# crismolav/ggnn

Measured on AMD Instinct MI355X. Metric: instances/sec (graphs/s) GGNN fwd+bwd, hidden=256 v=128 e=4 T=5, higher is better.
Workload: dtype fp32; 1 GPU; configs[2]: b=256 graphs/GPU, v=128, hidden=256, e=4 (C=8), T=5, fwd+bwd; global_batch=256, parallelism=dp1

## Files before the change

ggnn_amd/csrc/ggnn_api.hip:

```cpp
#include <hip/hip_runtime.h>
#include <stdint.h>
#include <string.h>

#include <algorithm>
#include <cmath>
#include <string>
#include <vector>

#include "../../include/ggnn.h"
#include "ggnn_common.h"
#include "k_gru.h"
#include "k_gru2.h"
#include "k_fused.h"
#include "k_prep.h"
#include "k_prop.h"
#include "k_optim.h"
#include "k_wgrad.h"
#include "k_head.h"
#include "k_decode.h"
#include "k_tree.h"
#include "k_proj.h"
#include "k_marg.h"
#include "k_lapl.h"
#include "k_tree_loss.h"
// ... 450 lines not shown
  Prof p(K_GRU_BWD, s);
  *nwg = (int)(c.N / (32 * RT));
  hipLaunchKernelGGL((k_gru_bwd<H, RT, PREC>), dim3(c.N / (32 * RT)), dim3(2 * H), 0, s, delta, hf, r, u, cc,
                     P<u16>(pk, PL.WcT), P<u16>(pk, PL.WgT), PL.loWc, PL.loWg, (ActT<PREC>*)dXT, dh_out,
                     (u16*)dzcT, (u16*)dzgT, dbc, dbg, c.N, gmax, bpart,
                     (H == 256 && c.V == 128) ? sbits : (const uint2*)nullptr, c.sdrop.scale);
}
long gru_bias_rows(const Cfg& c) { return (long)c.T * std::max<long>(c.N / 32, 1); }

#define DISPATCH_V(c, FN, H, PREC, ...)                 \
  do {                                                  \
    if ((c).V == 32) FN<32, H, PREC>(__VA_ARGS__);      \
    else if ((c).V == 64) FN<64, H, PREC>(__VA_ARGS__); \
    else FN<128, H, PREC>(__VA_ARGS__);                 \
  } while (0)
#define DISPATCH_VH(c, FN, PREC, ...)                                  \
  do {                                                                 \
    if ((c).H == 64) DISPATCH_V(c, FN, 64, PREC, __VA_ARGS__);         \
    else if ((c).H == 128) DISPATCH_V(c, FN, 128, PREC, __VA_ARGS__);  \
    else DISPATCH_V(c, FN, 256, PREC, __VA_ARGS__);                    \
  } while (0)
#define DISPATCH_RT(c, FN, H, PREC, ...)                                             \
  do {                                                                               \
    constexpr bool sp_ = Prec<PREC>::split;                                          \
    constexpr int mx_ = sp_ ? kSplitRT<FN##_tag>::value : kMaxRT<FN##_tag, H>::value; \
    const int rt_ = gru_rt(c, mx_);                                                  \
    if (mx_ >= 4 && rt_ == 4) FN<H, mx_ >= 4 ? 4 : 2, PREC>(__VA_ARGS__);            \
    else if (rt_ == 2) FN<H, 2, PREC>(__VA_ARGS__);                                  \
    else FN<H, 1, PREC>(__VA_ARGS__);                                                \
  } while (0)
#define DISPATCH_HRT(c, FN, PREC, ...)                                 \
  do {                                                                 \
    if ((c).H == 64) DISPATCH_RT(c, FN, 64, PREC, __VA_ARGS__);        \
    else if ((c).H == 128) DISPATCH_RT(c, FN, 128, PREC, __VA_ARGS__); \
    else DISPATCH_RT(c, FN, 256, PREC, __VA_ARGS__);                   \
  } while (0)

struct launch_gru_fwd_tag {};
struct launch_gru_bwd_tag {};
template <typename TAG, int H> struct kMaxRT { static constexpr int value = 4; };
template <typename TAG> struct kSplitRT { static constexpr int value = 2; };
template <> struct kMaxRT<launch_gru_bwd_tag, 256> { static constexpr int value = 2; };

void launch_pack(bool f16, const float* S, int ldS, long sS, int K, int N, int trans, u16* out, long sO, long lo,
                 int batch, hipStream_t s, Drop dr = Drop{0, 0, 0, 1.0f}, int t = 0) {
  const int total = (N / 32) * (K / 16) * 64;
  Prof p(K_PACK, s);
  if (f16)
    hipLaunchKernelGGL(k_pack_B<true>, dim3((total + 255) / 256, batch), dim3(256), 0, s, S, ldS, sS, K, N, trans, out,
                       sO, lo, dr, t);
  else
    hipLaunchKernelGGL(k_pack_B<false>, dim3((total + 255) / 256, batch), dim3(256), 0, s, S, ldS, sS, K, N, trans, out,
                       sO, lo, dr, t);
}
const Drop kNoDrop = {0, 0, 0, 1.0f};

template <int PREC>
int forward_impl(const Cfg& c, const void* pack, const void* adj, void* ws, bool tr, const float* h0, float* hT,
                 hipStream_t s) {
  typedef ActT<PREC> Act;
  constexpr bool SPLIT = Prec<PREC>::split;
  const WsL L = ws_layout(c, tr);
  const PackL PL = pack_layout(c);
  const AdjL AL = adj_layout(c);
  const long N = c.N, H = c.H;
  const bool dense = c.vin == c.V;
  const bool fused = fused_fwd(c);
  float* hf0 = tr ? P<float>(ws, L.hfT) : P<float>(ws, L.hf[0]);
  if (tr) {
    Prof p(K_IO, s);
    hipLaunchKernelGGL((k_stage_h0<Prec<PREC>::f16>), dim3((N + 63) / 64, H / 64), dim3(256), 0, s, h0, c.vin, c.V,
                       hf0, SPLIT ? (u16*)nullptr : P<u16>(ws, L.hb[0]), P<u16>(ws, L.hT), N, c.H);
  } else if (!dense || (!SPLIT && !fused)) {
    Prof p(K_IO, s);
    hipLaunchKernelGGL(k_pad_state, dim3(grid1d(N / 4 * H)), dim3(256), 0, s, h0, c.vin, c.V, c.H,
                       dense ? (float*)nullptr : hf0, SPLIT ? (u16*)nullptr : P<u16>(ws, L.hb[0]), N,
                       (int)Prec<PREC>::f16, kNoDrop, 0, (const uint32_t*)nullptr);
  }
  if (fused) {
    FusedFwdArgs fa;
    memset(&fa, 0, sizeof(fa));
    fa.Ab = P<u16>(adj, AL.Ab);
    const ChanL cl = chan_lists(c, adj, AL);
    fa.chl = cl.p;
    fa.chs = cl.stride;
    fa.Wp = P<u16>(pack, PL.wf(0));
    fa.wlo = PL.loW;
    fa.wstep = c.ed ? (long)(PL.szW / 2) : 0;
    fa.beta = P<float>(pack, PL.beta);
    fa.Wgp = P<u16>(pack, PL.Wg);
    fa.bg = P<float>(pack, PL.bg);
    fa.Wcp = P<u16>(pack, PL.Wc);
    fa.bc = P<float>(pack, PL.bc);
    fa.wlo_g = PL.loWg;
    fa.wlo_c = PL.loWc;
    fa.Xs = P<float>(ws, L.Xa);
    for (int t = 0; t <= c.T; ++t) {
      const float* hin = tr ? P<float>(ws, L.hfT + L.nh4 * t) : (t == 0 && dense) ? h0 : P<float>(ws, L.hf[t & 1]);
      fa.hf[t] = (t == c.T && dense) ? hT : (float*)hin;
    }
    if (tr) {
      fa.XT = P<u16>(ws, L.XT);
      fa.hT = P<u16>(ws, L.hT);
      fa.rhT = P<u16>(ws, L.rhT);
      fa.r = P<float>(ws, L.r);
      fa.u = P<float>(ws, L.u);
      fa.c = P<float>(ws, L.c);
      fa.sw = (long)(L.nhw / 2);
      fa.s4 = (long)(L.nh4 / 4);
    }
    fa.C = c.C;
    fa.T = c.T;
    fa.vsh = c.vsh;
    fa.sd = c.sdrop;
    fa.sbits = (tr && state_bits(c)) ? P<uint2>(ws, L.sbits) : nullptr;
    {
      Prof p(K_FWD_FUSED, s);
      hipLaunchKernelGGL(k_fwd_fused<PREC>, dim3(c.b), dim3(512), 0, s, fa);
    }
  } else
  for (int t = 0; t < c.T; ++t) {
    const float* hf_in = tr ? P<float>(ws, L.hfT + L.nh4 * t)
                            : (t == 0 && dense) ? h0 : P<float>(ws, L.hf[t & 1]);
    float* hf_out = (t + 1 == c.T && dense) ? hT
                    : tr                   ? P<float>(ws, L.hfT + L.nh4 * (t + 1))
                                           : P<float>(ws, L.hf[(t + 1) & 1]);
    const u16* hb_in = SPLIT ? nullptr : P<u16>(ws, L.hb[t & 1]);
    u16* hb_out = SPLIT ? nullptr : P<u16>(ws, L.hb[(t + 1) & 1]);
    const void* hs = SPLIT ? (const void*)hf_in : (const void*)hb_in;
    void* XT = tr ? P<void>(ws, L.XT + L.nhw * t) : nullptr;
    DISPATCH_VH(c, launch_prop_fwd, PREC, c, t, hs, P<u16>(adj, AL.Ab), chan_lists(c, adj, AL), PL, pack,
                P<void>(ws, L.Xa), XT, s);
    void* hTo = (tr && t + 1 < c.T) ? P<void>(ws, L.hT + L.nhw * (t + 1)) : nullptr;
    float* ro = tr ? P<float>(ws, L.r + L.nh4 * t) : nullptr;
    float* uo = tr ? P<float>(ws, L.u + L.nh4 * t) : nullptr;
    float* co = tr ? P<float>(ws, L.c + L.nh4 * t) : nullptr;
    void* rhT = tr ? P<void>(ws, L.rhT + L.nhw * t) : nullptr;
    DISPATCH_HRT(c, launch_gru_fwd, PREC, c, t, P<void>(ws, L.Xa), hb_in, hf_in, PL, pack, hf_out, hb_out, hTo, ro, uo,
                 co, rhT, s);
  }
  const float* hfin = tr ? P<float>(ws, L.hfT + L.nh4 * c.T) : P<float>(ws, L.hf[c.T & 1]);
  if (!dense) {
    Prof p(K_IO, s);
    hipLaunchKernelGGL(k_unpad_state, dim3(grid1d((long)c.b * c.vin * H)), dim3(256), 0, s, hfin, c.vin, c.V, c.H, hT,
                       (long)c.b, (const uint32_t*)nullptr);
  }
  LAUNCHCHK();
  return GGNN_OK;
}

template <int PREC>
int wgrad_impl(const Cfg& c, void* ws, int t0, int nt, float* dW, float* dWg, float* dWc, hipStream_t s);

struct Zeroer {
  hipStream_t s;
  ZeroJobs j;
  int n = 0;
  explicit Zeroer(hipStream_t st) : s(st) {}
  void add(float* p, long cnt) {
    if (cnt <= 0) return;
    j.p[n] = p, j.n[n] = cnt;
    if (++n == ZERO_MAXJ) flush();
  }
  void flush() {
    if (n) hipLaunchKernelGGL(k_zero_multi, dim3(256, n), dim3(256), 0, s, j);
    n = 0;
  }
  ~Zeroer() { flush(); }
};

template <int PREC>
int backward_impl(const Cfg& c, const void* pack, const void* adj, void* ws, const float* dhT, float* dh0, float* dW,
                  float* dbeta, float* dWg, float* dbg, float* dWc, float* dbc, hipStream_t s) {
  const WsL L = ws_layout(c, true);
  const PackL PL = pack_layout(c);
  const AdjL AL = adj_layout(c);
  const long N = c.N, H = c.H;
  const bool use_bias = (c.flags & GGNN_USE_EDGE_BIAS) != 0;
  if (H < 128) return fail(GGNN_EUNSUP, "weight gradients need hidden >= 128");

  const uint32_t* gmax = P<const uint32_t>(ws, L.gmax);
  {
    Prof p(K_IO, s);
    absmax(dhT, (long)c.b * c.vin * H, P<uint32_t>(ws, L.gmax), s);
  }
  float* dA = P<float>(ws, L.dA);
  float* dB = P<float>(ws, L.dB);
  const bool dense = c.vin == c.V;
  const uint2* sb = state_bits(c) ? P<const uint2>(ws, L.sbits) : nullptr;
  const bool in_place = dense && (!c.sd || sb);
  if (!in_place) {
    Prof p(K_IO, s);
    hipLaunchKernelGGL(k_pad_state, dim3(grid1d(N / 4 * H)), dim3(256), 0, s, dhT, c.vin, c.V, c.H, dA, (u16*)nullptr, N, 0,
                       c.sdrop, c.T - 1, gmax);
  }
  const long gb_stride = std::max<long>(N / 32, 1);
  int gb_nwg = 0;
  for (int t = c.T - 1; t >= 0; --t) {
    const bool first = t == c.T - 1 && in_place, last = t == 0 && dense;
    const float* delta = first ? dhT : dA;
    float* dh_out = last ? dh0 : dA;
// ... 99 lines not shown
  if (N % KC) return fail(GGNN_EUNSUP, "rows not divisible into weight-gradient chunks");
  a.KC = KC;
  a.nchunks = (int)(N / KC);
  {
    Prof p(K_WGRAD, s);
    if (KC % 64 != 0 || wp.KCt % 64 != 0) hipLaunchKernelGGL((k_wgrad<32, WP>), dim3(wgs), dim3(256), 0, s, a);
    else hipLaunchKernelGGL((k_wgrad<64, WP>), dim3(wgs), dim3(256), 0, s, a);
    hipLaunchKernelGGL(k_wgrad_reduce<128>, dim3(tiles * 16), dim3(256), 0, s, a);
  }
  LAUNCHCHK();
  return GGNN_OK;
}

#include "generic_path.h"

int pack_impl(const Cfg& c, void* pack, const unsigned char* chocc, const float* W, const float* beta,
              const float* Wg, const float* bg, const float* Wc, const float* bc, hipStream_t s) {
  const PackL L = pack_layout(c);
  const int H = c.H;
  PackJobs a;
  memset(&a, 0, sizeof(a));
  a.dr = c.edrop;
  a.chocc = chocc;
  int nb = 0;
  auto flush = [&]() {
    if (!a.count) return;
    a.blk_begin[a.count] = nb;
    Prof p(K_PACK, s);
    if (c.prec != PREC_BF16) hipLaunchKernelGGL(k_pack_multi<true>, dim3(nb), dim3(256), 0, s, a);
    else hipLaunchKernelGGL(k_pack_multi<false>, dim3(nb), dim3(256), 0, s, a);
    a.count = 0;
    nb = 0;
  };
  auto job = [&](const float* S, int ldS, long sS, int K, int N, int trans, void* out, long sO, long lo, int batch,
                 int t, int drop, int f8 = 0) {
    if (a.count == PACK_MAXJ) flush();
    PackJob& J = a.j[a.count];
    J.S = S; J.out = (u16*)out; J.sS = sS; J.sO = sO; J.lo_off = lo;
    J.total = (long)batch * (N / 32) * (K / 16) * 64;
    J.ldS = ldS; J.K = K; J.N = N; J.trans = trans; J.t = t; J.drop = drop; J.copy = 0; J.f8 = f8;
    a.blk_begin[a.count++] = nb;
    nb += (int)((J.total + 255) / 256);
  };
  auto copy = [&](const float* S, float* out, long n, int mode = 1, int t = 0, int drop = 0, uint32_t* bits = nullptr) {
    if (a.count == PACK_MAXJ) flush();
    PackJob& J = a.j[a.count];
    const int vec = mode == 2 && H % 4 == 0 && !(((uintptr_t)S | (uintptr_t)out) & 15);
    const long w32 = (H + 31) / 32;
    if (mode == 2 && vec) n = drop ? (long)c.C * w32 * (H / 4) : n / 4;
    else if (mode == 2 && drop) n = (long)c.C * w32 * H;
    J.S = S; J.out = (u16*)out; J.total = n; J.copy = mode; J.K = H; J.t = t; J.drop = drop; J.trans = vec;
    J.bits = drop ? bits : nullptr;
    a.blk_begin[a.count++] = nb;
    nb += (int)((n + 255) / 256);
  };
  if (L.fast) {
    for (int t = 0; t < (c.ed ? c.T : 1); ++t) {
      job(W, H, (long)H * H, H, H, 0, P<u16>(pack, L.wf(t)), (long)H * H, L.loW, c.C, t, c.ed);
      job(W, H, (long)H * H, H, H, 1, P<u16>(pack, L.wt(t)), (long)H * H, L.loW, c.C, t, c.ed, prop_f8(c));
    }
    job(Wg, 2 * H, 0, 2 * H, 2 * H, 0, P<u16>(pack, L.Wg), 0, L.loWg, 1, 0, 0);
    const int gf8 = c.prec == PREC_SPLIT ? 2 : 0;
    job(Wg, 2 * H, 0, 2 * H, 2 * H, 1, P<u16>(pack, L.WgT), 0, L.loWg, 1, 0, 0, gf8);
    job(Wc, H, 0, 2 * H, H, 0, P<u16>(pack, L.Wc), 0, L.loWc, 1, 0, 0);
    job(Wc, H, 0, H, 2 * H, 1, P<u16>(pack, L.WcT), 0, L.loWc, 1, 0, 0, gf8);
  }
  copy((c.flags & GGNN_USE_EDGE_BIAS) ? beta : nullptr, P<float>(pack, L.beta), (long)c.C * H);
  copy(bg, P<float>(pack, L.bg), 2L * H);
  copy(bc, P<float>(pack, L.bc), (long)H);
  for (int t = 0; t < (c.ed ? c.T : 1); ++t)
    copy(W, P<float>(pack, L.gw(t)), (long)c.C * H * H, 2, t, c.ed, c.ed ? P<uint32_t>(pack, L.gb(t)) : nullptr);
  copy(Wg, P<float>(pack, L.gWg), 4L * H * H);
  copy(Wc, P<float>(pack, L.gWc), 2L * H * H);
  flush();
  LAUNCHCHK();
  return GGNN_OK;
}

}

extern "C" {
#ifdef GGNN_TS
int ggnn_dbg_ts(void* host) { return (int)hipMemcpyFromSymbol(host, HIP_SYMBOL(g_ts), sizeof(g_ts)); }
int ggnn_dbg_clk(void* host) { return (int)hipMemcpyFromSymbol(host, HIP_SYMBOL(g_clk), sizeof(g_clk)); }
int ggnn_dbg_ts_clear(void) {
  static unsigned long long zero[sizeof(g_ts) / 8];
  return (int)hipMemcpyToSymbol(HIP_SYMBOL(g_ts), zero, sizeof(g_ts));
}
#endif

int ggnn_version(void) { return 4; }
const char* ggnn_last_error(void) { return g_err.c_str(); }

const char* ggnn_kernel_kind_name(int kind) {
  return (kind >= 0 && kind < GGNN_NUM_KERNEL_KINDS) ? kKindNames[kind] : "";
}

int ggnn_profile_begin(int max_launches) {
  if (max_launches < 1) return fail(GGNN_EINVAL, "profile_begin: max_launches < 1");
  for (hipEvent_t e : g_prof.ev)
    if (e) (void)hipEventDestroy(e);
  g_prof.ev.assign(2 * (size_t)max_launches, nullptr);
  g_prof.kind.assign(max_launches, 0);
  for (auto& e : g_prof.ev) HIPCHK(hipEventCreate(&e));
  g_prof.cap = max_launches;
  g_prof.used = 0;
  g_prof.on = true;
  return GGNN_OK;
}

int ggnn_profile_end(double* total_ms, int* launches) {
  if (!g_prof.on) return fail(GGNN_EINVAL, "profile_end without profile_begin");
  g_prof.on = false;
  for (int k = 0; k < GGNN_NUM_KERNEL_KINDS; ++k) {
    if (total_ms) total_ms[k] = 0.0;
    if (launches) launches[k] = 0;
  }
  for (int i = 0; i < g_prof.used; ++i) {
    HIPCHK(hipEventSynchronize(g_prof.ev[2 * i + 1]));
    float ms = 0.f;
    HIPCHK(hipEventElapsedTime(&ms, g_prof.ev[2 * i], g_prof.ev[2 * i + 1]));
    if (total_ms) total_ms[g_prof.kind[i]] += ms;
    if (launches) launches[g_prof.kind[i]] += 1;
  }
  const int overflow = g_prof.used >= g_prof.cap;
  g_prof.used = 0;
  return overflow ? fail(GGNN_EINVAL, "profile buffer full: raise max_launches") : GGNN_OK;
}

int ggnn_check_dims(const ggnn_dims* d) {
  Cfg c;
  return make_cfg(d, &c);
}

int ggnn_workspace_bytes(const ggnn_dims* d, int training, size_t* bytes) {
  Cfg c;
  int e = make_cfg(d, &c);
  if (e) return e;
  if (!bytes) return fail(GGNN_EINVAL, "bytes is NULL");
  *bytes = c.generic ? gen_ws_layout(c, training != 0).total : ws_layout(c, training != 0).total;
  return GGNN_OK;
}

int ggnn_adjacency_bytes(const ggnn_dims* d, size_t* bytes) {
  Cfg c;
  int e = make_cfg(d, &c);
  if (e) return e;
  if (!bytes) return fail(GGNN_EINVAL, "bytes is NULL");
  *bytes = c.generic ? gen_adj_layout(c).total : adj_layout(c).total;
  return GGNN_OK;
}

int ggnn_weight_pack_bytes(const ggnn_dims* d, size_t* bytes) {
  Cfg c;
  int e = make_cfg(d, &c);
  if (e) return e;
  if (!bytes) return fail(GGNN_EINVAL, "bytes is NULL");
  *bytes = pack_layout(c).total;
  return GGNN_OK;
}


int ggnn_pack_weights(const ggnn_dims* d, void* pack, const float* W, const float* beta, const float* Wg,
                      const float* bg, const float* Wc, const float* bc, ggnn_stream_t stream) {
  Cfg c;
  int e = make_cfg(d, &c);
// ... 862 lines not shown
```

ggnn_amd/csrc/ggnn_common.h:

```cpp
#pragma once

#include <hip/hip_runtime.h>
#include <stdint.h>

#include <type_traits>

typedef uint16_t u16;
typedef __bf16 bf16x8 __attribute__((ext_vector_type(8)));
typedef _Float16 f16x8 __attribute__((ext_vector_type(8)));
typedef float f32x16 __attribute__((ext_vector_type(16)));
typedef uint4 frag;
typedef unsigned int v2u32 __attribute__((ext_vector_type(2)));

#define DEV __device__ __forceinline__
#define HDI __host__ __device__ inline
#ifdef GGNN_TS
__device__ unsigned long long g_ts[4][2048 * 8];
#define TSMARK(k, i) do { if (threadIdx.x == 0) g_ts[k][blockIdx.x * 8 + (i)] = __builtin_amdgcn_s_memrealtime(); } while (0)
#define TSVAL(k, i, v) do { if (threadIdx.x == 0) g_ts[k][blockIdx.x * 8 + (i)] = (unsigned long long)(v); } while (0)
__device__ unsigned long long g_clk[4][2048 * 4];
#define TSCLK(k, e) do { if (threadIdx.x == 0) { \
    g_clk[k][blockIdx.x * 4 + 2 * (e)] = __builtin_amdgcn_s_memrealtime(); \
    g_clk[k][blockIdx.x * 4 + 2 * (e) + 1] = __builtin_amdgcn_s_memtime(); } } while (0)
#else
#define TSCLK(k, e) do {} while (0)
#define TSMARK(k, i) do {} while (0)
#define TSVAL(k, i, v) do {} while (0)
#endif

enum { PREC_BF16 = 0, PREC_F16 = 1, PREC_SPLIT = 2 };
template <int PREC> struct Prec {
  static constexpr bool split = PREC == PREC_SPLIT;
  static constexpr bool f16 = PREC != PREC_BF16;
};
template <int PREC>
using ActT = typename std::conditional<Prec<PREC>::split, float, u16>::type;

DEV u16 f2bf(float x) { return __builtin_bit_cast(u16, (__bf16)x); }
DEV float bf2f(u16 x) { return __uint_as_float(((uint32_t)x) << 16); }
DEV uint32_t pack2(float a, float b) { return (uint32_t)f2bf(a) | ((uint32_t)f2bf(b) << 16); }

template <bool F16> DEV u16 to_limb(float x) {
  if constexpr (F16) return __builtin_bit_cast(u16, (_Float16)x);
  else return f2bf(x);
}
template <bool F16> DEV float from_limb(u16 x) {
  if constexpr (F16) return (float)__builtin_bit_cast(_Float16, x);
  else return bf2f(x);
}
template <bool F16> DEV float lo_part(float x) { return x - from_limb<F16>(to_limb<F16>(x)); }
typedef float f32x2v __attribute__((ext_vector_type(2)));
typedef _Float16 f16x2v __attribute__((ext_vector_type(2)));
typedef __bf16 bf16x2v __attribute__((ext_vector_type(2)));
template <bool F16> DEV uint32_t pk(float a, float b) {
  const f32x2v v = {a, b};
  if constexpr (F16) return __builtin_bit_cast(uint32_t, __builtin_convertvector(v, f16x2v));
  else return __builtin_bit_cast(uint32_t, __builtin_convertvector(v, bf16x2v));
}
#ifndef GGNN_LIMB_MIX
#define GGNN_LIMB_MIX 1
#endif
template <bool F16, bool MIX = GGNN_LIMB_MIX> DEV uint32_t pk_lo(float a, float b) {
  if constexpr (F16 && MIX) {
    const uint32_t hi = pk<true>(a, b);
    uint32_t lo;
    asm("v_fma_mixlo_f16 %0, %1, 1.0, -%2 op_sel_hi:[0,0,1]" : "=v"(lo) : "v"(a), "v"(hi));
    asm("v_fma_mixhi_f16 %0, %1, 1.0, -%2 op_sel:[0,0,1] op_sel_hi:[0,0,1]\n\ts_nop 1" : "+v"(lo) : "v"(b), "v"(hi));
    return lo;
  }
  const f32x2v v = {a, b};
  f32x2v back;
  if constexpr (F16) back = __builtin_convertvector(__builtin_convertvector(v, f16x2v), f32x2v);
  else back = __builtin_convertvector(__builtin_convertvector(v, bf16x2v), f32x2v);
  const f32x2v lo = v - back;
  return pk<F16>(lo.x, lo.y);
}
template <bool F16> DEV frag pk8(const float* x) {
  return make_uint4(pk<F16>(x[0], x[1]), pk<F16>(x[2], x[3]), pk<F16>(x[4], x[5]), pk<F16>(x[6], x[7]));
}
DEV u16 lo_limb16(float v) {
  if constexpr (GGNN_LIMB_MIX) {
    const uint32_t hi = __builtin_bit_cast(u16, (_Float16)v);
    uint32_t lo;
    asm("v_fma_mixlo_f16 %0, %1, 1.0, -%2 op_sel_hi:[0,0,1]" : "=v"(lo) : "v"(v), "v"(hi));
    return (u16)lo;
  }
  return to_limb<true>(lo_part<true>(v));
}
template <int HALF> DEV float resid16(float x, uint32_t hpk) {
  if constexpr (GGNN_LIMB_MIX) {
    float lo;
    if constexpr (HALF == 0) asm("v_fma_mix_f32 %0, %1, 1.0, -%2 op_sel_hi:[0,0,1]" : "=v"(lo) : "v"(x), "v"(hpk));
    else asm("v_fma_mix_f32 %0, %1, 1.0, -%2 op_sel:[0,0,1] op_sel_hi:[0,0,1]" : "=v"(lo) : "v"(x), "v"(hpk));
    return lo;
  }
  return x - from_limb<true>((u16)(hpk >> (16 * HALF)));
}
template <bool F16, bool MIX = GGNN_LIMB_MIX> DEV frag pk8_lo(const float* x) {
  return make_uint4(pk_lo<F16, MIX>(x[0], x[1]), pk_lo<F16, MIX>(x[2], x[3]), pk_lo<F16, MIX>(x[4], x[5]),
                    pk_lo<F16, MIX>(x[6], x[7]));
}
template <bool F16> DEV float limb_elem(frag f, int j) {
  const uint32_t w = (j < 2) ? f.x : (j < 4) ? f.y : (j < 6) ? f.z : f.w;
  return from_limb<F16>((u16)((j & 1) ? (w >> 16) : (w & 0xffff)));
}

template <bool F16> DEV f32x16 mfma(frag a, frag b, f32x16 c) {
// ... 12 lines not shown
DEV float tanh_f(float x) { return 1.0f - 2.0f / (__expf(2.0f * x) + 1.0f); }
DEV constexpr int acc_row0(int r) { return (r & 3) + 8 * (r >> 2); }
DEV int acc_row(int r, int hh) { return acc_row0(r) + 4 * hh; }

template <bool F16> DEV frag acc_hi(const f32x16& a, int s) {
  float x[8];
#pragma unroll
  for (int j = 0; j < 8; ++j) x[j] = a[8 * s + j];
  return pk8<F16>(x);
}
template <bool F16, bool MIX = GGNN_LIMB_MIX> DEV frag acc_lo(const f32x16& a, int s) {
  float x[8];
#pragma unroll
  for (int j = 0; j < 8; ++j) x[j] = a[8 * s + j];
  return pk8_lo<F16, MIX>(x);
}

template <int PREC>
DEV void mma(f32x16& acc, frag ah, frag al, frag bh, frag bl) {
  if constexpr (Prec<PREC>::split) {
    acc = mfma<true>(al, bh, acc);
    acc = mfma<true>(ah, bl, acc);
  }
  acc = mfma<Prec<PREC>::f16>(ah, bh, acc);
}
template <int PREC>
DEV void mma_xa(f32x16& acc, frag a, frag bh, frag bl) {
  if constexpr (Prec<PREC>::split) acc = mfma<true>(a, bl, acc);
  acc = mfma<Prec<PREC>::f16>(a, bh, acc);
}
template <int PREC>
DEV void mma_xb(f32x16& acc, frag ah, frag al, frag b) {
  if constexpr (Prec<PREC>::split) acc = mfma<true>(al, b, acc);
  acc = mfma<Prec<PREC>::f16>(ah, b, acc);
}

constexpr int F8_Q = 7, F8_M = 11;
typedef int i32x8 __attribute__((ext_vector_type(8)));
DEV uint32_t pk4_bf8(float a, float b, float c, float d) {
  uint32_t w = (uint32_t)__builtin_amdgcn_cvt_pk_bf8_f32(a, b, 0, false);
  return (uint32_t)__builtin_amdgcn_cvt_pk_bf8_f32(c, d, (int)w, true);
}
DEV uint32_t pk4_fp8(float a, float b, float c, float d) {
  uint32_t w = (uint32_t)__builtin_amdgcn_cvt_pk_fp8_f32(a, b, 0, false);
  return (uint32_t)__builtin_amdgcn_cvt_pk_fp8_f32(c, d, (int)w, true);
}
DEV f32x16 mfma_f8corr(uint4 a0, uint4 a1, uint4 b0, uint4 b1, f32x16 c) {
  const i32x8 fa = {(int)a0.x, (int)a0.y, (int)a0.z, (int)a0.w, (int)a1.x, (int)a1.y, (int)a1.z, (int)a1.w};
  const i32x8 fb = {(int)b0.x, (int)b0.y, (int)b0.z, (int)b0.w, (int)b1.x, (int)b1.y, (int)b1.z, (int)b1.w};
  return __builtin_amdgcn_mfma_scale_f32_32x32x64_f8f6f4(fa, fb, c, 1, 0, 0, 127, 0, 127 - F8_Q - F8_M);
}

template <int NCH>
struct Swz {
  static constexpr int M = (NCH % 16 == 0) ? 15 : (NCH % 8 == 0) ? 7 : (NCH % 4 == 0) ? 3 : 0;
  static DEV int off(int row, int ch) { return row * NCH * 16 + ((ch ^ (row & M)) << 4); }
  static DEV int eoff(int row, int e) { return off(row, e >> 3) + ((e & 7) << 1); }
};

DEV uint4 ld16(const void* p) { return *(const uint4*)p; }
DEV void st16(void* p, uint4 v) { *(uint4*)p = v; }
DEV frag lds_frag(const char* img, int off) { return ld16(img + off); }
typedef short s16x4 __attribute__((ext_vector_type(4)));
DEV v2u32 lds_tr16(const char* p) {
  return __builtin_bit_cast(v2u32, __builtin_amdgcn_ds_read_tr16_b64_v4i16((__attribute__((address_space(3))) s16x4*)p));
}

template <bool NTEMP = false>
DEV void glds16_asm(const void* gsrc, const char* lds_dst) {
  unsigned keep;
  const unsigned dst = __builtin_amdgcn_readfirstlane((unsigned)(uintptr_t)lds_dst);
  if constexpr (NTEMP)
    asm volatile("s_mov_b32 %0, m0\n\ts_mov_b32 m0, %2\n\ts_nop 0\n\tglobal_load_lds_dwordx4 %1, off nt\n\ts_mov_b32 m0, %0"
                 : "=&s"(keep)
                 : "v"(gsrc), "s"(dst)
                 : "memory");
  else
    asm volatile("s_mov_b32 %0, m0\n\ts_mov_b32 m0, %2\n\ts_nop 0\n\tglobal_load_lds_dwordx4 %1, off\n\ts_mov_b32 m0, %0"
                 : "=&s"(keep)
                 : "v"(gsrc), "s"(dst)
                 : "memory");
}

template <int NCH, int R, int NT, int AUX = 0>
DEV void glds_tile(char* lds, const u16* src, int tid) {
  typedef Swz<NCH> S;
  constexpr int TOT = R * NCH;
  const int lane = tid & 63;
#pragma unroll
  for (int p = 0; p < (TOT + NT - 1) / NT; ++p) {
    const int qb = p * NT + (tid & ~63);
    if (qb < TOT) {
      const int q = qb + lane, row = q / NCH, pc = q % NCH;
      const u16* g = src + (row * NCH + (pc ^ (row & S::M))) * 8;
      __builtin_amdgcn_global_load_lds((const void*)g, (__attribute__((address_space(3))) void*)(lds + qb * 16), 16, 0, AUX);
    }
  }
}

template <int NCH, int R, int NT, int AUX = 0>
DEV void tile_ld(uint4 (&r)[(R * NCH + NT - 1) / NT], const u16* src, int tid) {
  typedef Swz<NCH> S;
  typedef unsigned int u32x4v __attribute__((ext_vector_type(4)));
  constexpr int TOT = R * NCH;
  asm volatile("" : "+v"(tid));
#pragma unroll
  for (int p = 0; p < (TOT + NT - 1) / NT; ++p) {
    const int q = p * NT + tid;
    if ((p + 1) * NT <= TOT || q < TOT) {
      const int row = q / NCH, pc = q % NCH;
      const u16* g = src + (row * NCH + (pc ^ (row & S::M))) * 8;
      if constexpr ((AUX & 2) != 0) r[p] = __builtin_bit_cast(uint4, __builtin_nontemporal_load((const u32x4v*)g));
      else r[p] = ld16(g);
    }
  }
}
template <int NCH, int R, int NT>
DEV void tile_st(char* lds, const uint4 (&r)[(R * NCH + NT - 1) / NT], int tid) {
  constexpr int TOT = R * NCH;
  asm volatile("" : "+v"(tid));
#pragma unroll
  for (int p = 0; p < (TOT + NT - 1) / NT; ++p) {
    const int q = p * NT + tid;
    if ((p + 1) * NT <= TOT || q < TOT) st16(lds + q * 16, r[p]);
  }
}

DEV frag frag_ld(const u16* base, int strip, int ks, int nks, int lane) {
  return ld16(base + ((size_t)(strip * nks + ks) * 64 + lane) * 8);
}

struct F2 { frag a, b; };
struct F4 { frag a, b, c, d; };
template <int KS, int D, int UNROLL = 0, typename LD, typename BODY>
DEV void b_pipeline(LD&& ld, BODY&& body) {
  static_assert(KS % D == 0, "k-steps must be a multiple of the pipeline depth");
  using FB = decltype(ld(0));
  FB ring[D];
#pragma unroll
  for (int p = 0; p < D; ++p) ring[p] = ld(p);
#pragma unroll (UNROLL == 0 ? KS / D : UNROLL)
  for (int k0 = 0; k0 < KS; k0 += D) {
#pragma unroll
    for (int p = 0; p < D; ++p) {
      body(k0 + p, ring[p]);
      ring[p] = ld(min(k0 + p + D, KS - 1));
      __builtin_amdgcn_sched_barrier(0);
    }
  }
}

template <int KS, int U, typename LD, typename BODY>
DEV void b_direct(LD&& ld, BODY&& body) {
#pragma unroll U
  for (int ks = 0; ks < KS; ++ks) body(ks, ld(ks));
}

DEV v2u32 quad_transpose4(uint32_t P0, uint32_t P1, int L) {
  const bool up = L & 2, odd = L & 1;
  const uint32_t Y = __builtin_amdgcn_update_dpp(0u, up ? P0 : P1, 0x4E, 0xF, 0xF, false);
  const uint32_t Q0 = up ? Y : P0, Q1 = up ? P1 : Y;
  const uint32_t S = odd ? ((Q0 & 0xFFFFu) | (Q1 << 16)) : ((Q0 >> 16) | (Q1 & 0xFFFF0000u));
  const uint32_t R = __builtin_amdgcn_update_dpp(0u, S, 0xB1, 0xF, 0xF, false);
  v2u32 w;
  if (!odd) {
    w.x = (Q0 & 0xFFFFu) | (R << 16);
    w.y = (Q1 & 0xFFFFu) | (R & 0xFFFF0000u);
  } else {
    w.x = (R & 0xFFFFu) | (Q0 & 0xFFFF0000u);
    w.y = (R >> 16) | (Q1 & 0xFFFF0000u);
  }
  return w;
}

struct Drop {
  uint32_t k0, k1;
  uint32_t thr;
  float scale;
  const uint32_t* kp;
};
DEV uint32_t dkey0(const Drop& d) { return d.kp ? d.kp[0] : d.k0; }
DEV uint32_t dkey1(const Drop& d) { return d.kp ? d.kp[1] : d.k1; }
DEV Drop drop_resolve(Drop d) {
  if (d.kp) {
    d.k0 = d.kp[0];
    d.k1 = d.kp[1];
  }
  d.kp = nullptr;
  return d;
}
DEV uint4 philox4x32_10(uint4 c, uint32_t k0, uint32_t k1) {
#pragma unroll
  for (int i = 0; i < 10; ++i) {
    const uint32_t lo0 = c.x * 0xD2511F53u, hi0 = __umulhi(c.x, 0xD2511F53u);
    const uint32_t lo1 = c.z * 0xCD9E8D57u, hi1 = __umulhi(c.z, 0xCD9E8D57u);
    c = make_uint4(hi1 ^ c.y ^ k0, lo1, hi0 ^ c.w ^ k1, lo0);
    k0 += 0x9E3779B9u;
    k1 += 0xBB67AE85u;
  }
  return c;
}
DEV uint32_t u4_get(const uint4& w, int j) { return j == 0 ? w.x : j == 1 ? w.y : j == 2 ? w.z : w.w; }
DEV uint4 state_words(const Drop& d, int g, int i, int k, int t) {
  return philox4x32_10(make_uint4((uint32_t)i >> 2, (uint32_t)k, (uint32_t)g, 0x80000000u | (uint32_t)t), dkey0(d), dkey1(d));
}
DEV uint4 edge_words(const Drop& d, int c, int i, int j, int t) {
  return philox4x32_10(make_uint4((uint32_t)i >> 2, (uint32_t)j, (uint32_t)c, (uint32_t)t), dkey0(d), dkey1(d));
}
DEV float drop_apply(const Drop& d, uint32_t w, float x) { return w < d.thr ? x * d.scale : 0.0f; }
DEV float gru_blend(float u, float h, float c) { return __builtin_fmaf(u, h, (1.0f - u) * c); }
DEV float gru_dzg_r(float x, float h, float r) { return x * h * r * (1.0f - r); }

DEV int gscale_exp(uint32_t gmax_bits) {
  const float m = __uint_as_float(gmax_bits);
  if (!(m > 0.0f) || !(m < 3.0e38f)) return 0;
  int e = ((int)(gmax_bits >> 23) & 0xff) - 127;
  if (e == -127) e = -126;
  return -max(-126, min(126, e));
}
DEV float gscale(const uint32_t* gmax) { return gmax ? __builtin_ldexpf(1.0f, gscale_exp(*gmax)) : 1.0f; }
DEV float gunscale(const uint32_t* gmax) { return gmax ? __builtin_ldexpf(1.0f, -gscale_exp(*gmax)) : 1.0f; }

typedef __amdgpu_buffer_rsrc_t rsrc_t;
constexpr int kNT = 2;
// ... 84 lines not shown
```

ggnn_amd/csrc/k_fused.h:

```cpp
#pragma once
#include "ggnn_common.h"
#include "k_gru2.h"

#define FUSED_MAXT 16
constexpr int kFusedAAux = kNT;
struct FusedFwdArgs {
  const u16* Ab;
  const int* chl;
  int chs;
  const u16* Wp;
  long wlo, wstep;
  const float* beta;
  const u16* Wgp;
  const float* bg;
  const u16* Wcp;
  const float* bc;
  long wlo_g, wlo_c;
  float* Xs;
  float* hf[FUSED_MAXT + 1];
  u16* XT;
  u16* hT;
  u16* rhT;
  float* r;
  float* u;
  float* c;
  long sw, s4;
  int C, T, vsh;
  Drop sd;
  uint2* sbits;
};

template <int PREC>
__global__ void __launch_bounds__(512) k_fwd_fused(FusedFwdArgs a) {
  const Drop sd = drop_resolve(a.sd);
  TSCLK(2, 0);
  using namespace gru2;
  constexpr bool SPLIT = Prec<PREC>::split, F16 = Prec<PREC>::f16;
  auto cput = [&](char* hi, char* lo, int off, const Chunk& v) {
    const float x[8] = {__uint_as_float(v.a.x), __uint_as_float(v.a.y), __uint_as_float(v.a.z), __uint_as_float(v.a.w),
                        __uint_as_float(v.b.x), __uint_as_float(v.b.y), __uint_as_float(v.b.z), __uint_as_float(v.b.w)};
    st16(hi + off, pk8<F16>(x));
    if constexpr (SPLIT) st16(lo + off, pk8_lo<true, false>(x));
  };
  constexpr int V = 128, VT = 4, ACH = V / 8;
  typedef Swz<ACH> SA;
  __shared__ __attribute__((aligned(16))) char smem[2 * IMG + 4 * SLOT];
  char* img_hi = smem;
  char* img_lo = smem + IMG;
  char* abuf = smem + 2 * IMG;
  auto slot_hi = [&](int u) { return smem + 2 * IMG + u * 2 * SLOT; };
  auto slot_lo = [&](int u) { return smem + 2 * IMG + u * 2 * SLOT + SLOT; };

  const int g = blockIdx.x;
  const long row0 = (long)g * R;
  const int C = a.C;
  const u16* ag = a.Ab + (long)g * C * V * V;
  const int* cl = a.chl + (long)g * a.chs;
  const int nc = cl[0];
  auto chan = [&](int i) { return cl[1 + i]; };
  float* xs = a.Xs + row0 * H;
  const rsrc_t rxs = mkrsrc(xs, R * H * 4);
  const rsrc_t wgh = mkrsrc(a.Wgp, 4 * H * H * 2), wgl = mkrsrc(a.Wgp + a.wlo_g, 4 * H * H * 2);
  const rsrc_t wch = mkrsrc(a.Wcp, 2 * H * H * 2), wcl = mkrsrc(a.Wcp + a.wlo_c, 2 * H * H * 2);

  {
    const int tid = threadIdx.x;
    const float* h0 = a.hf[0] + row0 * H;
    for (int q = tid; q < R * (H / 8); q += NT) {
      const int row = q & (R - 1), ch = q >> 7;
      const float4 x0 = *(const float4*)(h0 + row * H + ch * 8), x1 = *(const float4*)(h0 + row * H + ch * 8 + 4);
      const float x[8] = {x0.x, x0.y, x0.z, x0.w, x1.x, x1.y, x1.z, x1.w};
      st16(img_hi + koff(row, ch), pk8<F16>(x));
      if constexpr (SPLIT) st16(img_lo + koff(row, ch), pk8_lo<true, false>(x));
    }
  }
  if (nc > 0) glds_tile<ACH, V, NT, kFusedAAux>(abuf, ag + (long)chan(0) * V * V, (int)threadIdx.x);

  for (int t = 0; t < a.T; ++t) {
    __syncthreads();
    TSMARK(2, 0);
    int tid = threadIdx.x;
    asm volatile("" : "+v"(tid));
    const int lane = tid & 63, ns = tid >> 6, l32 = lane & 31, hh = lane >> 5;
    const int n = ns * 32 + l32;
    const int crow = crow_of(tid), cq = cq_of(tid);
    const int cso = koff(crow, cq);
    const int vo = (4 * hh * H + n) * 4;
    const int xvo_st = (ns * 4096 + lane) * 4;
    int xvo_ld;
    {
      const int it = crow >> 5, rr = crow & 31;
      const int r = (rr & 3) + 4 * (rr >> 3), h2 = (rr >> 2) & 1;
      xvo_ld = ((it * 16 + r) * 64 + h2 * 32 + 8 * cq) * 4;
    }
    auto xld = [&](int ck) {
      return Chunk{__builtin_bit_cast(uint4, __builtin_amdgcn_raw_buffer_load_b128(rxs, xvo_ld, ck * 16384, kNT)),
                   __builtin_bit_cast(uint4, __builtin_amdgcn_raw_buffer_load_b128(rxs, xvo_ld + 16, ck * 16384, kNT))};
    };
    const int vr = ((ns * KSG) * 64 + lane) * 16, vu = (((NS + ns) * KSG) * 64 + lane) * 16;
    const int vw = ((ns * KS) * 64 + lane) * 16;
    auto ldg = [&](int k) {
      return F4{wld(wgh, vr, k), SPLIT ? wld(wgl, vr, k) : frag{}, wld(wgh, vu, k), SPLIT ? wld(wgl, vu, k) : frag{}};
    };
    auto ldc = [&](int k) { return F2{wld(wch, vr, k), SPLIT ? wld(wcl, vr, k) : frag{}}; };
    const long wt = (long)t * a.wstep;
    const rsrc_t wfh = mkrsrc(a.Wp + wt, C * H * H * 2), wfl = mkrsrc(a.Wp + wt + a.wlo, C * H * H * 2);
    f32x16 accx[VT];
#pragma unroll
    for (int it = 0; it < VT; ++it) accx[it] = splat(0.f);
    for (int ci = 0; ci < nc; ++ci) {
      const int c = chan(ci);
      const float bb = a.beta[c * H + n];
      f32x16 accm[VT];
#pragma unroll
      for (int rt = 0; rt < VT; ++rt) accm[rt] = splat(bb);
      const int cw = c * H * H * 2;
      auto ldw = [&](int ks) {
        return F2{bld16(wfh, vw, cw + ks * 1024), SPLIT ? bld16(wfl, vw, cw + ks * 1024) : frag{}};
      };
      b_pipeline<KS, 2>(ldw, [&](int ks, const F2& w) {
#pragma unroll
        for (int rt = 0; rt < VT; ++rt) {
          const int off = koff(rt * 32 + l32, 2 * ks + hh);
          const frag ah = lds_frag(img_hi, off);
          mma<PREC>(accm[rt], ah, SPLIT ? lds_frag(img_lo, off) : ah, w.a, w.b);
        }
      });
      __syncthreads();
#pragma unroll
      for (int rt = 0; rt < VT; ++rt) {
        const frag mh0 = acc_hi<F16>(accm[rt], 0), mh1 = acc_hi<F16>(accm[rt], 1);
        const frag ml0 = SPLIT ? acc_lo<true, false>(accm[rt], 0) : mh0, ml1 = SPLIT ? acc_lo<true, false>(accm[rt], 1) : mh1;
#pragma unroll
        for (int it = 0; it < VT; ++it) {
          const frag a0 = lds_frag(abuf, SA::off(it * 32 + l32, 4 * rt + hh));
          const frag a1 = lds_frag(abuf, SA::off(it * 32 + l32, 4 * rt + 2 + hh));
          mma_xa<PREC>(accx[it], a0, mh0, ml0);
          mma_xa<PREC>(accx[it], a1, mh1, ml1);
        }
      }
      __syncthreads();
      if (ci + 1 < nc) glds_tile<ACH, V, NT, kFusedAAux>(abuf, ag + (long)chan(ci + 1) * V * V, tid);
    }
    TSMARK(2, 1);
#pragma unroll
    for (int it = 0; it < VT; ++it)
#pragma unroll
      for (int r = 0; r < 16; ++r) bst(rxs, accx[it][r], xvo_st, (it * 16 + r) * 256);
    if (a.XT) {
      u16* xt = a.XT + t * a.sw;
#pragma unroll
      for (int it = 0; it < VT; ++it)
#pragma unroll
        for (int q = 0; q < 4; ++q)
          st_col4w<PREC>(xt + wg_off(n, row0 + it * 32 + 4 * hh, H) + 8 * q, accx[it][4 * q],
                               accx[it][4 * q + 1], accx[it][4 * q + 2], accx[it][4 * q + 3]);
    }
    __syncthreads();
    TSMARK(2, 2);

    f32x16 ar[RT], au[RT];
    {
      const float br = a.bg[n], bu = a.bg[H + n];
#pragma unroll
      for (int rt = 0; rt < RT; ++rt) { ar[rt] = splat(br); au[rt] = splat(bu); }
    }
    Chunk st0 = xld(0), st1 = xld(1);
    F4 w0 = ldg(KS), w1 = ldg(KS + 1);
#pragma unroll
    for (int ks = 0; ks < KS; ks += 2) {
#pragma unroll
      for (int s = 0; s < 2; ++s) {
        const F4 w = s ? w1 : w0;
#pragma unroll
        for (int rt = 0; rt < RT; ++rt) {
          const int off = koff(rt * 32 + l32, 2 * (ks + s) + hh);
          const frag ah = lds_frag(img_hi, off), al = SPLIT ? lds_frag(img_lo, off) : ah;
          mma<PREC>(ar[rt], ah, al, w.a, w.b);
          mma<PREC>(au[rt], ah, al, w.c, w.d);
        }
        const int nk = ks + s + 2;
        const F4 nw = ldg(nk < KS ? KS + nk : nk - KS);
        if (s) w1 = nw;
        else w0 = nw;
        __builtin_amdgcn_sched_barrier(0);
      }
    }
    cput(slot_hi(0), slot_lo(0), cso, st0);
    st0 = xld(2);
    __syncthreads();
#pragma unroll
    for (int c = 0; c < NCHK; ++c) {
      if (c + 1 < NCHK) {
        cput(slot_hi((c + 1) & 1), slot_lo((c + 1) & 1), cso, (c & 1) ? st0 : st1);
        if (c + 3 < NCHK) {
          if (c & 1) st0 = xld(c + 3);
          else st1 = xld(c + 3);
        }
      }
#pragma unroll
      for (int s = 0; s < 2; ++s) {
        const int ks = 2 * c + s;
        const F4 w = s ? w1 : w0;
#pragma unroll
        for (int rt = 0; rt < RT; ++rt) {
          const int off = koff(rt * 32 + l32, 2 * s + hh);
          const frag ah = lds_frag(slot_hi(c & 1), off), al = SPLIT ? lds_frag(slot_lo(c & 1), off) : ah;
          mma<PREC>(ar[rt], ah, al, w.a, w.b);
          mma<PREC>(au[rt], ah, al, w.c, w.d);
        }
        const F4 nw = ldg(min(ks + 2, KS - 1));
        if (s) w1 = nw;
        else w0 = nw;
        __builtin_amdgcn_sched_barrier(0);
      }
      __syncthreads();
    }
    TSMARK(2, 3);
    st0 = xld(0);
    st1 = xld(1);

    {
      const rsrc_t rh32 = mkrsrc(a.hf[t] + row0 * H, R * H * 4);
      u16* rht = a.rhT ? a.rhT + t * a.sw : nullptr;
#pragma unroll
// ... 9 lines not shown
          if constexpr (SPLIT)
            hx = from_limb<true>(*(const u16*)(img_hi + eo)) + from_limb<true>(*(const u16*)(img_lo + eo));
          else
            hx = bld(rh32, vo, (rt * 32 + acc_row0(r)) * H * 4);
          rh[r] = rr * hx;
          *(u16*)(img_hi + eo) = to_limb<F16>(rh[r]);
          if constexpr (SPLIT) *(u16*)(img_lo + eo) = to_limb<true>(lo_part<true>(rh[r]));
        }
        if (a.r) {
#pragma unroll
          for (int q = 0; q < 4; ++q)
            gst4(a.r + t * a.s4 + row0 * H, qm_vo(hh, n, H), qm_so(rt, q, H),
                 make_float4(rv[4 * q], rv[4 * q + 1], rv[4 * q + 2], rv[4 * q + 3]));
        }
        if (rht) {
#pragma unroll
          for (int q = 0; q < 4; ++q)
            st_col4w<PREC>(rht + wg_off(n, row0 + rt * 32 + 4 * hh, H) + 8 * q, rh[4 * q], rh[4 * q + 1],
                                 rh[4 * q + 2], rh[4 * q + 3]);
        }
      }
    }
    cput(slot_hi(0), slot_lo(0), cso, st0);
    st0 = xld(2);
    __syncthreads();

    TSMARK(2, 4);
    f32x16 ac[RT];
    {
      const float b0 = a.bc[n];
#pragma unroll
      for (int rt = 0; rt < RT; ++rt) ac[rt] = splat(b0);
    }
    {
      F2 v0 = ldc(KS), v1 = ldc(KS + 1);
#pragma unroll
      for (int ks = 0; ks < KS; ks += 2) {
#pragma unroll
        for (int s = 0; s < 2; ++s) {
          const F2 w = s ? v1 : v0;
#pragma unroll
          for (int rt = 0; rt < RT; ++rt) {
            const int off = koff(rt * 32 + l32, 2 * (ks + s) + hh);
            const frag ah = lds_frag(img_hi, off);
            mma<PREC>(ac[rt], ah, SPLIT ? lds_frag(img_lo, off) : ah, w.a, w.b);
          }
          const int nk = ks + s + 2;
          const F2 nw = ldc(nk < KS ? KS + nk : nk - KS);
          if (s) v1 = nw;
          else v0 = nw;
          __builtin_amdgcn_sched_barrier(0);
        }
      }
      w0 = F4{v0.a, v0.b, v0.a, v0.b};
      w1 = F4{v1.a, v1.b, v1.a, v1.b};
    }
#pragma unroll
    for (int c = 0; c < NCHK; ++c) {
      if (c + 1 < NCHK) {
        cput(slot_hi((c + 1) & 1), slot_lo((c + 1) & 1), cso, (c & 1) ? st0 : st1);
        if (c + 3 < NCHK) {
          if (c & 1) st0 = xld(c + 3);
          else st1 = xld(c + 3);
        }
      }
#pragma unroll
      for (int s = 0; s < 2; ++s) {
        const int ks = 2 * c + s;
        const F4 w = s ? w1 : w0;
#pragma unroll
        for (int rt = 0; rt < RT; ++rt) {
          const int off = koff(rt * 32 + l32, 2 * s + hh);
          const frag ah = lds_frag(slot_hi(c & 1), off);
          mma<PREC>(ac[rt], ah, SPLIT ? lds_frag(slot_lo(c & 1), off) : ah, w.a, w.b);
        }
        const F2 nw = ldc(min(ks + 2, KS - 1));
        if (s) w1 = F4{nw.a, nw.b, nw.a, nw.b};
        else w0 = F4{nw.a, nw.b, nw.a, nw.b};
        __builtin_amdgcn_sched_barrier(0);
      }
      __syncthreads();
    }
    TSMARK(2, 5);
    if (t + 1 < a.T && nc > 0) glds_tile<ACH, V, NT, kFusedAAux>(abuf, ag + (long)chan(0) * V * V, tid);

    {
      const rsrc_t rhp = mkrsrc(a.hf[t] + row0 * H, R * H * 4);
      const rsrc_t ho = mkrsrc(a.hf[t + 1] + row0 * H, R * H * 4);
      const bool sav = a.u != nullptr;
      u16* hto = (a.hT && t + 1 < a.T) ? a.hT + (t + 1) * a.sw : nullptr;
      uint4 dw = make_uint4(0, 0, 0, 0);
      uint32_t kb[2] = {0u, 0u};
      float hp[RT][16];
#pragma unroll
      for (int rt = 0; rt < RT; ++rt)
#pragma unroll
        for (int r = 0; r < 16; ++r) hp[rt][r] = bld(rhp, vo, (rt * 32 + acc_row0(r)) * H * 4);
#pragma unroll
      for (int rt = 0; rt < RT; ++rt) {
        float hn[16], uv[16], cv[16];
#pragma unroll
        for (int r = 0; r < 16; ++r) {
          const int so = (rt * 32 + acc_row0(r)) * H * 4;
          const float cc = tanh_f(ac[rt][r]);
          const float u = au[rt][r];
          const float hprev = hp[rt][r];
          float x = u * hprev + (1.0f - u) * cc;
          if (sd.thr) {
            if ((r & 3) == 0) {
              dw = state_words(sd, g, rt * 32 + acc_row0(r) + 4 * hh, n, t);
            }
            x = drop_apply(sd, u4_get(dw, r & 3), x);
            kb[rt >> 1] |= (uint32_t)(u4_get(dw, r & 3) < sd.thr) << ((rt & 1) * 16 + r);
          }
          hn[r] = x;
          bst(ho, x, vo, so);
          uv[r] = u;
          cv[r] = cc;
        }
        if (sav) {
#pragma unroll
          for (int q = 0; q < 4; ++q) {
            gst4(a.u + t * a.s4 + row0 * H, qm_vo(hh, n, H), qm_so(rt, q, H),
                 make_float4(uv[4 * q], uv[4 * q + 1], uv[4 * q + 2], uv[4 * q + 3]));
            gst4(a.c + t * a.s4 + row0 * H, qm_vo(hh, n, H), qm_so(rt, q, H),
                 make_float4(cv[4 * q], cv[4 * q + 1], cv[4 * q + 2], cv[4 * q + 3]));
          }
        }
#pragma unroll
        for (int q = 0; q < 4; ++q) {
          const int eo = koff(rt * 32 + 8 * q + 4 * hh + (l32 & 3), n >> 3) + (n & 4) * 2;
          const v2u32 wh = quad_transpose4(pk<F16>(hn[4 * q], hn[4 * q + 1]), pk<F16>(hn[4 * q + 2], hn[4 * q + 3]), l32 & 3);
          *(uint2*)(img_hi + eo) = make_uint2(wh.x, wh.y);
          if constexpr (SPLIT) {
            const v2u32 wl = quad_transpose4(pk_lo<true, false>(hn[4 * q], hn[4 * q + 1]), pk_lo<true, false>(hn[4 * q + 2], hn[4 * q + 3]), l32 & 3);
            *(uint2*)(img_lo + eo) = make_uint2(wl.x, wl.y);
          }
        }
        if (hto) {
#pragma unroll
          for (int q = 0; q < 4; ++q)
            st_col4w<PREC>(hto + wg_off(n, row0 + rt * 32 + 4 * hh, H) + 8 * q, hn[4 * q], hn[4 * q + 1],
                                 hn[4 * q + 2], hn[4 * q + 3]);
        }
      }
      if (a.sbits && sd.thr) a.sbits[((long)t * gridDim.x + g) * NT + tid] = make_uint2(kb[0], kb[1]);
    }
    TSMARK(2, 6);
  }
  TSCLK(2, 1);
}
```

Before: 111,300 graphs/s.

## Prefetch next channel's weights and bias across channel loop in fused forward

Restructures the per-channel message loop in the fused forward kernel so the first two weight k-steps and the beta bias for the next channel are loaded during the adjacency-mixing phase of the current channel, instead of at the start of each channel. Channel list pointer and stride become kernel arguments rather than struct fields, and the first two channel ids are hoisted. Adjacency tile loads can now use an inline-asm global-to-LDS path. The goal is to hide global-load latency at channel boundaries, at the cost of more live registers and an explicit vmcnt(0) wait. It also adds optional timestamp instrumentation.

```diff
diff --git a/ggnn_amd/csrc/ggnn_api.hip b/ggnn_amd/csrc/ggnn_api.hip
--- a/ggnn_amd/csrc/ggnn_api.hip
+++ b/ggnn_amd/csrc/ggnn_api.hip
@@ -556,8 +556,6 @@
     memset(&fa, 0, sizeof(fa));
     fa.Ab = P<u16>(adj, AL.Ab);
     const ChanL cl = chan_lists(c, adj, AL);
-    fa.chl = cl.p;
-    fa.chs = cl.stride;
     fa.Wp = P<u16>(pack, PL.wf(0));
     fa.wlo = PL.loW;
     fa.wstep = c.ed ? (long)(PL.szW / 2) : 0;
@@ -590,7 +588,7 @@
     fa.sbits = (tr && state_bits(c)) ? P<uint2>(ws, L.sbits) : nullptr;
     {
       Prof p(K_FWD_FUSED, s);
-      hipLaunchKernelGGL(k_fwd_fused<PREC>, dim3(c.b), dim3(512), 0, s, fa);
+      hipLaunchKernelGGL(k_fwd_fused<PREC>, dim3(c.b), dim3(512), 0, s, fa, cl.p, cl.stride);
     }
   } else
   for (int t = 0; t < c.T; ++t) {
@@ -856,6 +854,7 @@
 extern "C" {
 #ifdef GGNN_TS
 int ggnn_dbg_ts(void* host) { return (int)hipMemcpyFromSymbol(host, HIP_SYMBOL(g_ts), sizeof(g_ts)); }
+int ggnn_dbg_tsc(void* host) { return (int)hipMemcpyFromSymbol(host, HIP_SYMBOL(g_tsc), sizeof(g_tsc)); }
 int ggnn_dbg_clk(void* host) { return (int)hipMemcpyFromSymbol(host, HIP_SYMBOL(g_clk), sizeof(g_clk)); }
 int ggnn_dbg_ts_clear(void) {
   static unsigned long long zero[sizeof(g_ts) / 8];
diff --git a/ggnn_amd/csrc/ggnn_common.h b/ggnn_amd/csrc/ggnn_common.h
--- a/ggnn_amd/csrc/ggnn_common.h
+++ b/ggnn_amd/csrc/ggnn_common.h
@@ -22,7 +22,11 @@
 #define TSCLK(k, e) do { if (threadIdx.x == 0) { \
     g_clk[k][blockIdx.x * 4 + 2 * (e)] = __builtin_amdgcn_s_memrealtime(); \
     g_clk[k][blockIdx.x * 4 + 2 * (e) + 1] = __builtin_amdgcn_s_memtime(); } } while (0)
+__device__ unsigned long long g_tsc[2048 * 8];
+#define TSCH(ci, nc, i) do { if (threadIdx.x == 0 && (ci) == max((nc) - 2, 0)) \
+    g_tsc[blockIdx.x * 8 + (i)] = __builtin_amdgcn_s_memrealtime(); } while (0)
 #else
+#define TSCH(ci, nc, i) do {} while (0)
 #define TSCLK(k, e) do {} while (0)
 #define TSMARK(k, i) do {} while (0)
 #define TSVAL(k, i, v) do {} while (0)
@@ -201,7 +205,7 @@
                  : "memory");
 }
 
-template <int NCH, int R, int NT, int AUX = 0>
+template <int NCH, int R, int NT, int AUX = 0, bool ASM = false>
 DEV void glds_tile(char* lds, const u16* src, int tid) {
   typedef Swz<NCH> S;
   constexpr int TOT = R * NCH;
@@ -209,10 +213,11 @@
 #pragma unroll
   for (int p = 0; p < (TOT + NT - 1) / NT; ++p) {
     const int qb = p * NT + (tid & ~63);
-    if (qb < TOT) {
+    if ((p + 1) * NT <= TOT || qb < TOT) {
       const int q = qb + lane, row = q / NCH, pc = q % NCH;
       const u16* g = src + (row * NCH + (pc ^ (row & S::M))) * 8;
-      __builtin_amdgcn_global_load_lds((const void*)g, (__attribute__((address_space(3))) void*)(lds + qb * 16), 16, 0, AUX);
+      if constexpr (ASM) glds16_asm<(AUX & 2) != 0>((const void*)g, lds + qb * 16);
+      else __builtin_amdgcn_global_load_lds((const void*)g, (__attribute__((address_space(3))) void*)(lds + qb * 16), 16, 0, AUX);
     }
   }
 }
@@ -259,6 +264,20 @@
 #pragma unroll
   for (int p = 0; p < D; ++p) ring[p] = ld(p);
 #pragma unroll (UNROLL == 0 ? KS / D : UNROLL)
+  for (int k0 = 0; k0 < KS; k0 += D) {
+#pragma unroll
+    for (int p = 0; p < D; ++p) {
+      body(k0 + p, ring[p]);
+      ring[p] = ld(min(k0 + p + D, KS - 1));
+      __builtin_amdgcn_sched_barrier(0);
+    }
+  }
+}
+
+template <int KS, int D, typename FB, typename LD, typename BODY>
+DEV void b_pipeline_pre(FB (&ring)[D], LD&& ld, BODY&& body) {
+  static_assert(KS % D == 0, "k-steps must be a multiple of the pipeline depth");
+#pragma unroll
   for (int k0 = 0; k0 < KS; k0 += D) {
 #pragma unroll
     for (int p = 0; p < D; ++p) {
diff --git a/ggnn_amd/csrc/k_fused.h b/ggnn_amd/csrc/k_fused.h
--- a/ggnn_amd/csrc/k_fused.h
+++ b/ggnn_amd/csrc/k_fused.h
@@ -6,8 +6,6 @@
 constexpr int kFusedAAux = kNT;
 struct FusedFwdArgs {
   const u16* Ab;
-  const int* chl;
-  int chs;
   const u16* Wp;
   long wlo, wstep;
   const float* beta;
@@ -31,7 +29,7 @@
 };
 
 template <int PREC>
-__global__ void __launch_bounds__(512) k_fwd_fused(FusedFwdArgs a) {
+__global__ void __launch_bounds__(512) k_fwd_fused(FusedFwdArgs a, const int* __restrict__ chl, int chs) {
   const Drop sd = drop_resolve(a.sd);
   TSCLK(2, 0);
   using namespace gru2;
@@ -55,9 +53,10 @@
   const long row0 = (long)g * R;
   const int C = a.C;
   const u16* ag = a.Ab + (long)g * C * V * V;
-  const int* cl = a.chl + (long)g * a.chs;
+  const int* cl = chl + (long)g * chs;
   const int nc = cl[0];
   auto chan = [&](int i) { return cl[1 + i]; };
+  const int c0 = nc > 0 ? chan(0) : 0, c1 = nc > 1 ? chan(1) : c0;
   float* xs = a.Xs + row0 * H;
   const rsrc_t rxs = mkrsrc(xs, R * H * 4);
   const rsrc_t wgh = mkrsrc(a.Wgp, 4 * H * H * 2), wgl = mkrsrc(a.Wgp + a.wlo_g, 4 * H * H * 2);
@@ -74,7 +73,7 @@
       if constexpr (SPLIT) st16(img_lo + koff(row, ch), pk8_lo<true, false>(x));
     }
   }
-  if (nc > 0) glds_tile<ACH, V, NT, kFusedAAux>(abuf, ag + (long)chan(0) * V * V, (int)threadIdx.x);
+  if (nc > 0) glds_tile<ACH, V, NT, kFusedAAux>(abuf, ag + (long)c0 * V * V, (int)threadIdx.x);
 
   for (int t = 0; t < a.T; ++t) {
     __syncthreads();
@@ -108,17 +107,45 @@
     f32x16 accx[VT];
 #pragma unroll
     for (int it = 0; it < VT; ++it) accx[it] = splat(0.f);
+    int c = c0, cn = c1;
+    auto ldw_at = [&](int cc, int ks) {
+      const int cw = cc * H * H * 2;
+      return F2{bld16(wfh, vw, cw + ks * 1024), SPLIT ? bld16(wfl, vw, cw + ks * 1024) : frag{}};
+    };
+    auto landed = [&](F2 (&r)[2], float& b) {
+      typedef unsigned int u32x4v __attribute__((ext_vector_type(4)));
+#pragma unroll
+      for (int p = 0; p < 2; ++p) {
+        u32x4v x = __builtin_bit_cast(u32x4v, r[p].a);
+        asm volatile("" : "+v"(x));
+        r[p].a = __builtin_bit_cast(frag, x);
+        if constexpr (SPLIT) {
+          u32x4v y = __builtin_bit_cast(u32x4v, r[p].b);
+          asm volatile("" : "+v"(y));
+          r[p].b = __builtin_bit_cast(frag, y);
+        }
+      }
+      asm volatile("" : "+v"(b));
+    };
+    F2 ring[2] = {};
+    float bb = 0.f;
+    if (nc > 0) {
+      bb = a.beta[c * H + n];
+      ring[0] = ldw_at(c, 0);
+      ring[1] = ldw_at(c, 1);
+      landed(ring, bb);
+    }
     for (int ci = 0; ci < nc; ++ci) {
-      const int c = chan(ci);
-      const float bb = a.beta[c * H + n];
+      const int cnn = chan(ci + 2 < nc ? ci + 2 : 0);
+      TSCH(ci, nc, 0);
+#ifdef GGNN_TS
+      asm volatile("" : "+v"(bb));
+#endif
       f32x16 accm[VT];
 #pragma unroll
       for (int rt = 0; rt < VT; ++rt) accm[rt] = splat(bb);
-      const int cw = c * H * H * 2;
-      auto ldw = [&](int ks) {
-        return F2{bld16(wfh, vw, cw + ks * 1024), SPLIT ? bld16(wfl, vw, cw + ks * 1024) : frag{}};
-      };
-      b_pipeline<KS, 2>(ldw, [&](int ks, const F2& w) {
+      TSCH(ci, nc, 1);
+      b_pipeline_pre<KS, 2>(ring, [&](int ks) { return ldw_at(c, ks); }, [&](int ks, const F2& w) {
 #pragma unroll
         for (int rt = 0; rt < VT; ++rt) {
           const int off = koff(rt * 32 + l32, 2 * ks + hh);
@@ -126,7 +153,13 @@
           mma<PREC>(accm[rt], ah, SPLIT ? lds_frag(img_lo, off) : ah, w.a, w.b);
         }
       });
+      TSCH(ci, nc, 2);
+      asm volatile("s_waitcnt vmcnt(0)" ::: "memory");
       __syncthreads();
+      bb = a.beta[cn * H + n];
+      ring[0] = ldw_at(cn, 0);
+      ring[1] = ldw_at(cn, 1);
+      __builtin_amdgcn_sched_barrier(0);
 #pragma unroll
       for (int rt = 0; rt < VT; ++rt) {
         const frag mh0 = acc_hi<F16>(accm[rt], 0), mh1 = acc_hi<F16>(accm[rt], 1);
@@ -140,7 +173,16 @@
         }
       }
       __syncthreads();
-      if (ci + 1 < nc) glds_tile<ACH, V, NT, kFusedAAux>(abuf, ag + (long)chan(ci + 1) * V * V, tid);
+      TSCH(ci, nc, 3);
+      landed(ring, bb);
+      if (ci + 1 < nc) {
+        int td = tid;
+        asm volatile("" : "+v"(td));
+        glds_tile<ACH, V, NT, kFusedAAux, true>(abuf, ag + (long)cn * V * V, td);
+      }
+      TSCH(ci, nc, 4);
+      c = cn;
+      cn = cnn;
     }
     TSMARK(2, 1);
 #pragma unroll
@@ -316,7 +358,7 @@
       __syncthreads();
     }
     TSMARK(2, 5);
-    if (t + 1 < a.T && nc > 0) glds_tile<ACH, V, NT, kFusedAAux>(abuf, ag + (long)chan(0) * V * V, tid);
+    if (t + 1 < a.T && nc > 0) glds_tile<ACH, V, NT, kFusedAAux>(abuf, ag + (long)c0 * V * V, tid);
 
     {
       const rsrc_t rhp = mkrsrc(a.hf[t] + row0 * H, R * H * 4);
```

Measured after the change: 111,900 graphs/s, median of 6. About the same (+0.6%).
